# FerrisMind/candle-video

Hardware: AMD Instinct MI355X
Metric: frames/sec end-to-end LTX-Video-2B 512x768x97; DiT step ms; VAE decode ms (higher is better)
Workload: dtype bf16; 1 GPU; LTX-Video-0.9.8-2B-distilled 512x768x97, 7 steps (configs.rs:223-240), untiled VAE decode; preset=0.9.8-2b-distilled, denoise_steps=7, parallelism=replicas x1 (no data-path collective)

## Files before the change

candle-video_amd/csrc/conv_halo.hip:

```cpp
#include <type_traits>
#include "gemm_common.h"
#include "options.h"

#ifndef HALO_WIDE_EPI
#define HALO_WIDE_EPI 1
#endif
#ifndef HALO_LOADERS
#define HALO_LOADERS 4
#endif
#ifndef HALO_PABL
#define HALO_PABL 0
#endif
#ifndef HALO_ABL
#define HALO_ABL 0
#endif

#ifdef HALO_TRACE
__device__ unsigned long long g_halo_trace[16384 * 8];
extern "C" int ltx_dbg_halo_trace(unsigned long long* out, int n) { return hipMemcpyFromSymbol(out, HIP_SYMBOL(g_halo_trace), (size_t)n * 8) == hipSuccess ? 0 : -1; }
#define HSTAMP(i) do { if (threadIdx.x == 0 && blockIdx.x < 16384) g_halo_trace[blockIdx.x * 8 + (i)] = __builtin_amdgcn_s_memrealtime(); } while (0)
#define HCYC(i) do { if (threadIdx.x == 0 && blockIdx.x < 16384) g_halo_trace[blockIdx.x * 8 + (i)] = __builtin_amdgcn_s_memtime(); } while (0)
#else
#define HSTAMP(i) do { } while (0)
#define HCYC(i) do { } while (0)
#endif

namespace {

constexpr int ROWB = 128;
constexpr int PH = 16, PW = 16, HW = PW + 2, HROWS = (PH + 2) * HW;
constexpr int A_PIECES = (HROWS + 7) / 8;
constexpr int A_STAGE = A_PIECES * 1024;
constexpr uint32_t OOB = 0x80000000u;
template <int I, int N, typename F> __device__ __forceinline__ void sfor_h(F&& f) {
    if constexpr (I < N) { f(std::integral_constant<int, I>{}); sfor_h<I + 1, N>(f); }
}

__device__ __forceinline__ int swz_h(int row, int chunk) { return row * ROWB + ((chunk ^ ((row >> 1) & 7)) << 4); }

extern __shared__ __attribute__((aligned(16))) unsigned char halo_smem[];

template <int BN, int WGM, int WGN, int EPI, bool PIPE>
__global__ __launch_bounds__(WGM * WGN * 64) void conv_halo_kernel(const GemmArgs g) {
    constexpr int NW = WGM * WGN, BM = PH * PW, WM = BM / WGM, WN = BN / WGN, FM = WM / 16, FN = BN == 64 ? 3 : WN / 16;
    static_assert((NW == 8 || (NW == 4 && PIPE)) && WM % 16 == 0 && WN % 16 == 0, "wave layout");
    constexpr int NTHR = NW * 64;
    constexpr int NL = (HALO_LOADERS == 4 && (BN == 128 || (BN == 64 && PIPE))) ? 4 : NW;
    constexpr int AJ = (A_PIECES + NL - 1) / NL, BJ = BN / (8 * NL);
    constexpr int B_STAGE = BN * ROWB;
    constexpr int A_ST = PIPE ? AJ * NL * 1024 : A_STAGE;
    static_assert(!PIPE || (NL == 4 && (BN == 128 || BN == 64)), "pipelined form: four loader waves, 128-wide tile (or conv_out's 64-wide one)");
    unsigned char* Abuf = halo_smem;
    unsigned char* Bbuf = halo_smem + 2 * A_ST;
    HSTAMP(0);
#ifndef HALO_NO_KERNARG_BATCH
    asm volatile("" :: "s"(g.A), "s"(g.W), "s"(g.C), "s"(g.bias), "s"(g.resid), "s"(g.N), "s"(g.K), "s"(g.Cin), "s"(g.T), "s"(g.H), "s"(g.Wd), "s"(g.ntaps), "s"(g.pad_t),
                 "s"(g.ldc), "s"(g.ldr), "s"(gridDim.x));
#endif

    const int tid = threadIdx.x, lane = tid & 63, wave = __builtin_amdgcn_readfirstlane(tid >> 6);
    const int wm = wave / WGN, wn = wave % WGN;
    const int lwave = wave & (NL - 1);
    const bool loader = wave < NL;
    const int frow = lane & 15, fq = lane >> 4;

    const int ntn = (g.N + BN - 1) / BN, pwn = (g.Wd + PW - 1) / PW, phn = (g.H + PH - 1) / PH;
    int bid = blockIdx.x;
    {
        const int nblk = (int)gridDim.x, q = nblk >> 3, r = nblk & 7, x = bid & 7, i = bid >> 3;
        bid = (x < r ? x * (q + 1) : r * (q + 1) + (x - r) * q) + i;
    }
#ifdef HALO_SAME_TILE
    bid = bid % ntn;
#endif
    const int nt = bid % ntn; int rr = bid / ntn;
    const int px = rr % pwn; rr /= pwn;
    const int py = rr % phn; const int bt = rr / phn;
    const int t = bt % g.T, b = bt / g.T;
    const int y0 = py * PH, x0 = px * PW, n0 = nt * BN;

    const bf16_t* __restrict__ A = reinterpret_cast<const bf16_t*>(g.A);
    const bf16_t* __restrict__ W = reinterpret_cast<const bf16_t*>(g.W);
    const int64_t frame_elems = (int64_t)g.H * g.Wd * g.Cin;
    const int tt0 = t - g.pad_t < 0 ? 0 : (t - g.pad_t > g.T - 1 ? g.T - 1 : t - g.pad_t);
    const __amdgpu_buffer_rsrc_t ra = __builtin_amdgcn_make_buffer_rsrc(const_cast<bf16_t*>(A + ((int64_t)b * g.T + tt0) * frame_elems), 0, (int)OOB, 0x00020000);
    const __amdgpu_buffer_rsrc_t rw = __builtin_amdgcn_make_buffer_rsrc(const_cast<bf16_t*>(W), 0, (int)OOB, 0x00020000);
    auto dma = [&](__amdgpu_buffer_rsrc_t r, uint32_t voff, uint32_t soff, unsigned char* lds) {
        __builtin_amdgcn_raw_ptr_buffer_load_lds(r, (__attribute__((address_space(3))) void*)lds, 16, (int)voff, (int)soff, 0, 0);
    };

    const int lr = lane >> 3, pc = lane & 7;
    uint32_t a_voff[AJ], b_voff[BJ];
#pragma unroll
    for (int j = 0; j < AJ; ++j) {
        const int hrow = (j * NL + lwave) * 8 + lr;
        const int hy = hrow / HW, hx = hrow - hy * HW;
        const int lc = pc ^ ((hx >> 1) & 7);
        const int y = y0 - 1 + hy, x = x0 - 1 + hx;
        const bool ok = hrow < HROWS && y >= 0 && y < g.H && x >= 0 && x < g.Wd;
        a_voff[j] = ok ? (uint32_t)(((y * g.Wd + x) * g.Cin + lc * 8) * 2) : OOB;
    }
#pragma unroll
    for (int j = 0; j < BJ; ++j) {
        const int row = (j * NL + lwave) * 8 + lr;
        const int lc = pc ^ ((row >> 1) & 7);
        b_voff[j] = n0 + row < g.N ? (uint32_t)((((n0 + row) * g.K) + lc * 8) * 2) : OOB;
    }
    const int KC = g.Cin / 64;
    const int KT = g.ntaps / 9;
    const int G = KT * KC;
    const uint32_t frame_bytes = (uint32_t)g.H * g.Wd * g.Cin * 2u;
    auto issue_a = [&](int grp, int j) {
        const int piece = j * NL + lwave;
        if (!loader || piece >= A_PIECES) return;
        const int it = grp / KC, kc = grp - it * KC;
        int tt = t + it - g.pad_t; tt = tt < 0 ? 0 : (tt > g.T - 1 ? g.T - 1 : tt);
        const uint32_t soff = (uint32_t)(tt - tt0) * frame_bytes + (uint32_t)kc * 128u;
        dma(ra, a_voff[j], soff, Abuf + (grp & 1) * A_ST + piece * 1024);
    };
    auto issue_b = [&](int grp, int hw, int buf) {
        if (!loader) return;
        const int it = grp / KC, kc = grp - it * KC;
        const uint32_t soff = ((uint32_t)(it * 9 + hw) * (uint32_t)g.N * (uint32_t)g.K + (uint32_t)kc * 64u) * 2u;
#pragma unroll
        for (int j = 0; j < BJ; ++j) dma(rw, b_voff[j], soff, Bbuf + buf * B_STAGE + (j * NL + lwave) * 1024);
    };

    f32x4 acc[FM][FN];
#pragma unroll
    for (int i = 0; i < FM; ++i)
#pragma unroll
        for (int j = 0; j < FN; ++j) acc[i][j] = (f32x4){0.f, 0.f, 0.f, 0.f};

    int rowbase[FM], colpart[3][2];
#pragma unroll
    for (int fm = 0; fm < FM; ++fm) rowbase[fm] = ((wm * FM + fm) * HW + frow) * ROWB;
#pragma unroll
    for (int iw = 0; iw < 3; ++iw)
#pragma unroll
        for (int kb = 0; kb < 2; ++kb) colpart[iw][kb] = iw * ROWB + (((kb * 4 + fq) ^ (((frow + iw) >> 1) & 7)) << 4);

    if constexpr (PIPE) {
        auto issue_a_p = [&](int grp, int j) {
            if (!loader) return;
            const int piece = j * NL + lwave;
            const int it = grp / KC, kc = grp - it * KC;
            int tt = t + it - g.pad_t; tt = tt < 0 ? 0 : (tt > g.T - 1 ? g.T - 1 : tt);
            const uint32_t soff = (uint32_t)(tt - tt0) * frame_bytes + (uint32_t)kc * 128u;
            const bool live = grp < G && piece < A_PIECES;
            if ((HALO_PABL & 2) && grp > 0) return;
            dma(ra, live ? a_voff[j] : OOB, live ? soff : 0u, Abuf + (grp & 1) * A_ST + piece * 1024);
        };
        auto issue_b_p = [&](int grp, int hw) {
            if (!loader) return;
            const int it = grp / KC, kc = grp - it * KC;
            const bool live = grp < G;
            const uint32_t soff = live ? ((uint32_t)(it * 9 + hw) * (uint32_t)g.N * (uint32_t)g.K + (uint32_t)kc * 64u) * 2u : 0u;
            if ((HALO_PABL & 2) && (grp > 0 || hw > 1)) return;
#pragma unroll
            for (int j = 0; j < BJ; ++j) dma(rw, live ? b_voff[j] : OOB, soff, Bbuf + (hw % 3) * B_STAGE + (j * NL + lwave) * 1024);
        };
        Chunk16 w0[FN], a0[FM], w1[FN], a1[FM];
        bool frags_once = false;
        auto read_frags = [&](int grp, int hw, int kb, Chunk16 (&wf)[FN], Chunk16 (&af)[FM]) {
            if (HALO_PABL & 4) {
                if (frags_once) {
#pragma unroll
                    for (int f = 0; f < FN; ++f) asm volatile("" : "+v"(wf[f].u));
#pragma unroll
                    for (int f = 0; f < FM; ++f) asm volatile("" : "+v"(af[f].u));
                    return;
                }
            }
            const int ih = hw / 3, iw = hw % 3;
            const unsigned char* As = Abuf + (grp & 1) * A_ST;
            const unsigned char* Bs = Bbuf + (hw % 3) * B_STAGE;
#pragma unroll
            for (int f = 0; f < FN; ++f) wf[f].u = *reinterpret_cast<const u32x4*>(Bs + swz_h(wn * WN + f * 16 + frow, kb * 4 + fq));
#pragma unroll
            for (int fm = 0; fm < FM; ++fm) af[fm].u = *reinterpret_cast<const u32x4*>(As + rowbase[fm] + colpart[iw][kb] + ih * HW * ROWB);
        };
        auto mma_all = [&](Chunk16 (&wf)[FN], Chunk16 (&af)[FM]) {
#pragma unroll
            for (int fm = 0; fm < FM; ++fm)
#pragma unroll
                for (int fn = 0; fn < FN; ++fn) acc[fm][fn] = Mma<bf16_t>::run(wf[fn], af[fm], acc[fm][fn]);
        };
        auto interleave = [&]() {
#pragma unroll
            for (int i = 0; i < FN + FM; ++i) {
                __builtin_amdgcn_sched_group_barrier(0x100, 1, 0);
                __builtin_amdgcn_sched_group_barrier(0x008, FM * FN / (FN + FM), 0);
            }
        };
#pragma unroll
        for (int j = 0; j < AJ; ++j) issue_a_p(0, j);
        issue_b_p(0, 0); issue_b_p(0, 1);
        asm volatile("s_waitcnt vmcnt(0)" ::: "memory");
        __syncthreads();
        HSTAMP(1); HCYC(5);
        read_frags(0, 0, 0, w0, a0);
        if (HALO_PABL & 4) { read_frags(0, 0, 1, w1, a1); frags_once = true; }
        auto step_p = [&](int grp, auto hw_tag) {
            constexpr int hw = decltype(hw_tag)::value;
            constexpr int RPS = (AJ + 5) / 6;
            constexpr int na = (hw + 1) * RPS <= AJ ? RPS : (hw * RPS < AJ ? AJ - hw * RPS : 0);
            if (hw + 2 < 9) issue_b_p(grp, hw + 2); else issue_b_p(grp + 1, hw + 2 - 9);
#pragma unroll
            for (int rr = 0; rr < na; ++rr) issue_a_p(grp + 1, hw * RPS + rr);
            read_frags(grp, hw, 1, w1, a1);
            mma_all(w0, a0);
            interleave();
            if ((HALO_PABL & 9) == 9 || (HALO_PABL & 3) == 3) {}
            else if (HALO_PABL & 1) asm volatile("s_waitcnt vmcnt(%0)" :: "n"(BJ + na) : "memory");
            else if (HALO_PABL & (8 | 2)) asm volatile("s_barrier" ::: "memory");
            else
            asm volatile("s_waitcnt vmcnt(%0)\n\ts_barrier" :: "n"(BJ + na) : "memory");
            if (hw + 1 < 9) read_frags(grp, hw + 1, 0, w0, a0); else read_frags(grp + 1, 0, 0, w0, a0);
            mma_all(w1, a1);
            interleave();
        };
        if constexpr (NW == 4) {
            auto mfma = [&](f32x4& c, const Chunk16& w, const Chunk16& a_) {
                asm volatile("v_mfma_f32_16x16x32_bf16 %0, %1, %2, %0" : "+a"(c) : "v"(w.u), "v"(a_.u));
            };
            const uint32_t nk2 = (uint32_t)g.N * (uint32_t)g.K * 2u;
            auto a_soff_of = [&](int it, int kc) {
                int tt = t + it - g.pad_t; tt = tt < 0 ? 0 : (tt > g.T - 1 ? g.T - 1 : tt);
                return (uint32_t)(tt - tt0) * frame_bytes + (uint32_t)kc * 128u;
            };
            int it_n = KC > 1 ? 0 : 1, kc_n = KC > 1 ? 1 : 0;
            uint32_t w_cur = 0u;
            for (int grp = 0; grp < G; ++grp) {
                const bool live_n = grp + 1 < G;
                const uint32_t a_next = live_n ? a_soff_of(it_n, kc_n) : 0u;
                const uint32_t w_next = live_n ? ((uint32_t)(it_n * 9) * (uint32_t)g.N * (uint32_t)g.K + (uint32_t)kc_n * 64u) * 2u : 0u;
                unsigned char* const a_dst = Abuf + ((grp + 1) & 1) * A_ST;
                sfor_h<0, 9>([&](auto hw_tag) {
                    constexpr int hw = decltype(hw_tag)::value;
                    constexpr int RPS = (AJ + 5) / 6;
                    constexpr int na = (hw + 1) * RPS <= AJ ? RPS : (hw * RPS < AJ ? AJ - hw * RPS : 0);
                    constexpr int NP = BJ + na, NM = FM * FN;
                    constexpr int h2 = hw + 2 < 9 ? hw + 2 : hw + 2 - 9;
                    const bool w_live = hw + 2 < 9 ? true : live_n;
                    const uint32_t w_soff = (hw + 2 < 9 ? w_cur : w_next) + (uint32_t)h2 * nk2;
                    auto read_one = [&](int rg, int rh, int kb, auto idx_tag, Chunk16 (&wf)[FN], Chunk16 (&af)[FM]) {
                        constexpr int idx = decltype(idx_tag)::value;
                        if (HALO_PABL & 4) return;
                        const int ih = rh / 3, iw = rh % 3;
                        if constexpr (idx < FN) wf[idx].u = *reinterpret_cast<const u32x4*>(Bbuf + (rh % 3) * B_STAGE + swz_h(wn * WN + idx * 16 + frow, kb * 4 + fq));
                        else af[idx - FN].u = *reinterpret_cast<const u32x4*>(Abuf + (rg & 1) * A_ST + rowbase[idx - FN] + colpart[iw][kb] + ih * HW * ROWB);
                    };
                    auto piece = [&](auto i_tag) {
                        constexpr int i = decltype(i_tag)::value;
                        if constexpr (i < BJ) {
                            if (!((HALO_PABL & 2) && (grp > 0 || hw > 1)))
                                dma(rw, w_live ? b_voff[i] : OOB, w_live ? w_soff : 0u, Bbuf + (h2 % 3) * B_STAGE + (i * NL + lwave) * 1024);
                        } else {
                            constexpr int j = hw * RPS + (i - BJ);
                            const bool live = live_n && j * NL + lwave < A_PIECES;
                            if (!(HALO_PABL & 2)) dma(ra, live ? a_voff[j] : OOB, live ? a_next : 0u, a_dst + (j * NL + lwave) * 1024);
                        }
                    };
                    sfor_h<0, NM>([&](auto m_tag) {
                        constexpr int mi = decltype(m_tag)::value;
                        if constexpr (mi % 2 == 0 && mi / 2 < FN + FM) read_one(grp, hw, 1, std::integral_constant<int, mi / 2>{}, w1, a1);
                        if constexpr (mi % 2 == 1 && (mi / 2) % (16 / NP > 0 ? 16 / NP : 1) == 0 && (mi / 2) / (16 / NP > 0 ? 16 / NP : 1) < NP)
                            piece(std::integral_constant<int, (mi / 2) / (16 / NP > 0 ? 16 / NP : 1)>{});
                        mfma(acc[mi / FN][mi % FN], w0[mi % FN], a0[mi / FN]);
                        __builtin_amdgcn_sched_barrier(0);
                    });
                    if ((HALO_PABL & 9) == 9 || (HALO_PABL & 3) == 3) {}
                    else if (HALO_PABL & 1) asm volatile("s_waitcnt vmcnt(%0)" :: "n"(BJ + na) : "memory");
                    else if (HALO_PABL & (8 | 2)) asm volatile("s_barrier" ::: "memory");
                    else asm volatile("s_waitcnt vmcnt(%0)\n\ts_barrier" :: "n"(BJ + na) : "memory");
                    __builtin_amdgcn_sched_barrier(0);
                    sfor_h<0, NM>([&](auto m_tag) {
                        constexpr int mi = decltype(m_tag)::value;
                        if constexpr (mi % 2 == 0 && mi / 2 < FN + FM) {
                            if (hw + 1 < 9) read_one(grp, hw + 1, 0, std::integral_constant<int, mi / 2>{}, w0, a0);
                            else read_one(grp + 1, 0, 0, std::integral_constant<int, mi / 2>{}, w0, a0);
                        }
                        mfma(acc[mi / FN][mi % FN], w1[mi % FN], a1[mi / FN]);
                        __builtin_amdgcn_sched_barrier(0);
                    });
                });
                w_cur = w_next;
                if (++kc_n == KC) { kc_n = 0; ++it_n; }
            }
            asm volatile("s_nop 15\n\ts_nop 15" ::: "memory");
        } else
        for (int grp = 0; grp < G; ++grp) {
            step_p(grp, std::integral_constant<int, 0>{}); step_p(grp, std::integral_constant<int, 1>{}); step_p(grp, std::integral_constant<int, 2>{});
            step_p(grp, std::integral_constant<int, 3>{}); step_p(grp, std::integral_constant<int, 4>{}); step_p(grp, std::integral_constant<int, 5>{});
            step_p(grp, std::integral_constant<int, 6>{}); step_p(grp, std::integral_constant<int, 7>{}); step_p(grp, std::integral_constant<int, 8>{});
        }
        HCYC(6); HSTAMP(2);
        asm volatile("s_waitcnt vmcnt(0)" ::: "memory");
        __syncthreads();
    } else {
#pragma unroll
    for (int j = 0; j < AJ; ++j) issue_a(0, j);
    issue_b(0, 0, 0);
    asm volatile("s_waitcnt vmcnt(0)" ::: "memory");
    __syncthreads();

    auto step = [&](int grp, auto hw_tag, int buf) {
        constexpr int hw = decltype(hw_tag)::value;
        constexpr int ih = hw / 3, iw = hw % 3;
        if (!(HALO_ABL & 4)) { if (hw < 8) issue_b(grp, hw + 1, buf ^ 1); else if (grp + 1 < G) issue_b(grp + 1, 0, buf ^ 1); }
        constexpr int RPS = (AJ + 8) / 9;
        if (!(HALO_ABL & 4) && grp + 1 < G) {
#pragma unroll
            for (int rr = 0; rr < RPS; ++rr) if (hw * RPS + rr < AJ) issue_a(grp + 1, hw * RPS + rr);
        }
        const unsigned char* As = Abuf + (grp & 1) * A_ST;
        const unsigned char* Bs = Bbuf + buf * B_STAGE;
#pragma unroll
        for (int kb = 0; kb < 2; ++kb) {
            Chunk16 af[FM], wf[FN];
#pragma unroll
            for (int f = 0; f < FN; ++f) {
                if ((HALO_ABL & 2) && f > 0) { wf[f].u = wf[0].u + (u32x4){(uint32_t)f, 0u, 0u, 0u}; continue; }
                wf[f].u = *reinterpret_cast<const u32x4*>(Bs + swz_h(wn * WN + f * 16 + frow, kb * 4 + fq));
            }
            int fr_ = frow; asm volatile("" : "+v"(fr_));
            const int cp = BN == 256 ? iw * ROWB + (((kb * 4 + fq) ^ (((fr_ + iw) >> 1) & 7)) << 4) : colpart[iw][kb];
            af[0].u = *reinterpret_cast<const u32x4*>(As + rowbase[0] + cp + ih * HW * ROWB);
#pragma unroll
            for (int fm = 0; fm < FM; ++fm) {
                if ((HALO_ABL & 1) && fm + 1 < FM) af[fm + 1].u = af[0].u + (u32x4){(uint32_t)fm, 0u, 0u, 0u};
                else
                if (fm + 1 < FM) af[fm + 1].u = *reinterpret_cast<const u32x4*>(As + rowbase[fm + 1] + cp + ih * HW * ROWB);
#pragma unroll
                for (int fn = 0; fn < FN; ++fn) acc[fm][fn] = Mma<bf16_t>::run(wf[fn], af[fm], acc[fm][fn]);
            }
        }
#pragma unroll
        for (int kb = 0; kb < 2; ++kb) {
            __builtin_amdgcn_sched_group_barrier(0x100, FN + 1, 0);
#pragma unroll
            for (int fm = 0; fm < FM; ++fm) {
                if (fm + 1 < FM) __builtin_amdgcn_sched_group_barrier(0x100, 1, 0);
                __builtin_amdgcn_sched_group_barrier(0x008, FN, 0);
            }
        }
        asm volatile("s_waitcnt vmcnt(0)" ::: "memory");
        __syncthreads();
    };
    for (int grp = 0; grp < G; ++grp) {
        const int p = grp & 1;
        step(grp, std::integral_constant<int, 0>{}, p);
        step(grp, std::integral_constant<int, 1>{}, p ^ 1);
        step(grp, std::integral_constant<int, 2>{}, p);
        step(grp, std::integral_constant<int, 3>{}, p ^ 1);
        step(grp, std::integral_constant<int, 4>{}, p);
        step(grp, std::integral_constant<int, 5>{}, p ^ 1);
        step(grp, std::integral_constant<int, 6>{}, p);
        step(grp, std::integral_constant<int, 7>{}, p ^ 1);
        step(grp, std::integral_constant<int, 8>{}, p);
    }

    }
    constexpr bool WIDE = HALO_WIDE_EPI && (EPI == EPI_BIAS || EPI == EPI_RESID);
    if constexpr (WIDE) {
        if (g.wide_epi) {
            constexpr int CPR = BN / 8, XM = 15, RPP = 64 / CPR;
            const int64_t frame_row0 = ((int64_t)b * g.T + t) * g.H * g.Wd;
            const __amdgpu_buffer_rsrc_t rr = __builtin_amdgcn_make_buffer_rsrc(
                const_cast<bf16_t*>(reinterpret_cast<const bf16_t*>(g.resid ? g.resid : g.C) + frame_row0 * g.ldr), 0, (int)OOB, 0x00020000);
            auto row_m = [&](int row, bool& inside) {
                const int y = y0 + (row >> 4), x = x0 + (row & 15);
                inside = y < g.H && x < g.Wd;
                return ((b * g.T + t) * g.H + y) * g.Wd + x;
            };
            if constexpr (EPI == EPI_RESID) {
                for (int pi = wave; pi < BM / RPP; pi += NW) {
                    const int row = pi * RPP + lane / CPR, pc = lane % CPR;
                    const int lc = pc ^ (row & XM);
                    bool inside; const int m = row_m(row, inside);
                    dma(rr, inside ? (uint32_t)((((int64_t)m - frame_row0) * g.ldr + n0 + lc * 8) * 2) : OOB, 0u, halo_smem + pi * 1024);
                }
                asm volatile("s_waitcnt vmcnt(0)" ::: "memory");
            }
            float bias4[FN][4];
#pragma unroll
            for (int fn = 0; fn < FN; ++fn) {
#pragma unroll
                for (int i = 0; i < 4; ++i) bias4[fn][i] = 0.f;
            }
            if (g.bias) {
#pragma unroll
                for (int fn = 0; fn < FN; ++fn) load4<bf16_t>(reinterpret_cast<const bf16_t*>(g.bias) + n0 + wn * WN + fn * 16 + 4 * fq, bias4[fn]);
            }
            __syncthreads();
#pragma unroll
            for (int fm = 0; fm < FM; ++fm) {
                const int row = (wm * FM + fm) * 16 + frow;
#pragma unroll
                for (int fn = 0; fn < FN; ++fn) {
                    const int col = wn * WN + fn * 16 + 4 * fq;
                    unsigned char* slot = halo_smem + row * (CPR * 16) + (((col >> 3) ^ (row & XM)) << 4) + ((col >> 2) & 1) * 8;
                    float v[4] = {acc[fm][fn][0], acc[fm][fn][1], acc[fm][fn][2], acc[fm][fn][3]};
                    {
#pragma unroll
                        for (int i = 0; i < 4; ++i) v[i] += bias4[fn][i];
                    }
                    if constexpr (EPI == EPI_RESID) {
                        float r[4];
                        load4<bf16_t>(reinterpret_cast<const bf16_t*>(slot), r);
#pragma unroll
                        for (int i = 0; i < 4; ++i) v[i] += r[i];
                    }
                    store4<bf16_t>(reinterpret_cast<bf16_t*>(slot), v);
                }
            }
            __syncthreads();
            bf16_t* Cb = reinterpret_cast<bf16_t*>(g.C);
            float pn_sc[8], pn_sh[8];
            bool pn_mod = false;
            if constexpr (EPI == EPI_BIAS) {
                if (g.pn_on && g.pn_scale) {
                    pn_mod = true;
                    const int c0 = tid % CPR;
                    const f32x4* scp = reinterpret_cast<const f32x4*>(g.pn_scale + (int64_t)b * g.pn_mod_stride + c0 * 8);
                    const f32x4* shp = reinterpret_cast<const f32x4*>(g.pn_shift + (int64_t)b * g.pn_mod_stride + c0 * 8);
                    const f32x4 s0 = scp[0], s1 = scp[1], h0 = shp[0], h1 = shp[1];
#pragma unroll
                    for (int j = 0; j < 4; ++j) { pn_sc[j] = 1.0f + s0[j]; pn_sc[4 + j] = 1.0f + s1[j]; pn_sh[j] = h0[j]; pn_sh[4 + j] = h1[j]; }
                }
            }
            for (int id = tid; id < BM * CPR; id += NTHR) {
                const int row = id / CPR, c = id - row * CPR;
                bool inside; const int m = row_m(row, inside);
                Chunk16 cc; cc.u = *reinterpret_cast<const u32x4*>(halo_smem + row * (CPR * 16) + ((c ^ (row & XM)) << 4));
                if constexpr (EPI == EPI_BIAS) {
                    if (g.pn_on) {
                        float f[8]; chunk_to_f32<bf16_t>(cc, f);
                        float ss = 0.f;
#pragma unroll
                        for (int j = 0; j < 8; ++j) ss += f[j] * f[j];
#pragma unroll
                        for (int o = CPR / 2; o > 0; o >>= 1) ss += __shfl_xor(ss, o);
                        const float rinv = __builtin_amdgcn_rsqf(ss * (1.0f / (float)BN) + g.pn_eps);
#pragma unroll
                        for (int j = 0; j < 8; ++j) {
                            float n = f[j] * rinv;
                            if (pn_mod) n = n * pn_sc[j] + pn_sh[j];
                            if (g.pn_act == 1) n = silu_f(n);
                            f[j] = n;
                        }
                        f32_to_chunk<bf16_t>(f, cc);
                    }
                }
                if (!inside) continue;
                *reinterpret_cast<u32x4*>(Cb + (int64_t)m * g.ldc + n0 + c * 8) = cc.u;
            }
#ifdef HALO_TRACE
            HSTAMP(3); asm volatile("s_waitcnt vmcnt(0)" ::: "memory"); HSTAMP(4);
            if (threadIdx.x == 0 && blockIdx.x < 16384) { unsigned hw; asm volatile("s_getreg_b32 %0, hwreg(HW_REG_HW_ID)" : "=s"(hw)); g_halo_trace[blockIdx.x * 8 + 7] = hw; }
#endif
            return;
        }
    }
    if constexpr (EPI == EPI_S2D) {
        float bias4[FN][4];
#pragma unroll
        for (int fn = 0; fn < FN; ++fn) {
#pragma unroll
            for (int i = 0; i < 4; ++i) bias4[fn][i] = 0.f;
        }
        if (g.bias) {
#pragma unroll
            for (int fn = 0; fn < FN; ++fn) {
                int nb = n0 + wn * WN + fn * 16 + 4 * fq; nb = nb < g.N ? nb : g.N - 4;
                load4<bf16_t>(reinterpret_cast<const bf16_t*>(g.bias) + nb, bias4[fn]);
            }
        }
        const int npass = (t == 0 && g.s2_st > 1) ? 2 : 1;
        for (int pass = 0; pass < npass; ++pass) {
#pragma unroll
            for (int fm = 0; fm < FM; ++fm) {
                int y = y0 + wm * FM + fm, x = x0 + frow;
                const bool inside = y < g.H && x < g.Wd;
                y = y < g.H ? y : g.H - 1; x = x < g.Wd ? x : g.Wd - 1;
                float res[FN][4];
#pragma unroll
                for (int fn = 0; fn < FN; ++fn) {
                    int nb = n0 + wn * WN + fn * 16 + 4 * fq; nb = nb < g.N ? nb : g.N - 4;
                    s2d_residual<bf16_t>(g, b, t, y, x, nb, pass, res[fn]);
                }
                if (!inside) continue;
#pragma unroll
                for (int fn = 0; fn < FN; ++fn) {
                    const int nb = n0 + wn * WN + fn * 16 + 4 * fq;
                    if (nb >= g.N) continue;
                    float v[4];
#pragma unroll
                    for (int i = 0; i < 4; ++i) v[i] = acc[fm][fn][i] + bias4[fn][i];
                    s2d_store<bf16_t>(g, b, t, y, x, nb, pass, v, res[fn]);
                }
            }
        }
    } else if constexpr (EPI == EPI_D2S || EPI == EPI_UNPATCH || EPI == EPI_BIAS || EPI == EPI_D2S_G) {
        float bias4[FN][4];
#pragma unroll
        for (int fn = 0; fn < FN; ++fn) {
            const int nb = n0 + wn * WN + fn * 16 + 4 * fq;
#pragma unroll
            for (int i = 0; i < 4; ++i) bias4[fn][i] = 0.f;
        }
        if (g.bias) {
#pragma unroll
            for (int fn = 0; fn < FN; ++fn) {
                int nb = n0 + wn * WN + fn * 16 + 4 * fq; nb = nb < g.N ? nb : g.N - 4;
                load4<bf16_t>(reinterpret_cast<const bf16_t*>(g.bias) + nb, bias4[fn]);
            }
        }
        const bool d2s_res = EPI == EPI_D2S && g.resid != nullptr;
        GemmArgs gs = g; gs.bias = nullptr; gs.resid = nullptr;
        constexpr int FC = FM * FN > 16 ? 2 : FM;
#pragma unroll
        for (int f0 = 0; f0 < FM; f0 += FC) {
            bf16_t raw[FC][FN][4];
            if constexpr (EPI == EPI_D2S) {
                if (d2s_res) {
                    const int nsub = g.d2s_sp ? 4 : 8;
#pragma unroll
                    for (int fc = 0; fc < FC; ++fc) {
                        int y = y0 + wm * FM + f0 + fc, x = x0 + frow;
                        y = y < g.H ? y : g.H - 1; x = x < g.Wd ? x : g.Wd - 1;
                        const int m = ((b * g.T + t) * g.H + y) * g.Wd + x;
                        const bf16_t* xr = reinterpret_cast<const bf16_t*>(g.resid) + (int64_t)m * g.Cin;
#pragma unroll
                        for (int fn = 0; fn < FN; ++fn) {
                            int nb = n0 + wn * WN + fn * 16 + 4 * fq; nb = nb < g.N ? nb : g.N - 4;
                            const int sidx = nb / g.Cf, co = nb - sidx * g.Cf;
#pragma unroll
                            for (int i = 0; i < 4; ++i) raw[fc][fn][i] = xr[((co + i) % g.Cr) * nsub + sidx];
                        }
                    }
                }
            }
#pragma unroll
            for (int fc = 0; fc < FC; ++fc) {
                const int fm = f0 + fc;
                const int y = y0 + wm * FM + fm, x = x0 + frow;
                if (y >= g.H || x >= g.Wd) continue;
                const int m = ((b * g.T + t) * g.H + y) * g.Wd + x;
#pragma unroll
                for (int fn = 0; fn < FN; ++fn) {
                    const int nb = n0 + wn * WN + fn * 16 + 4 * fq;
                    if (nb >= g.N) continue;
                    float v[4];
#pragma unroll
                    for (int i = 0; i < 4; ++i) v[i] = acc[fm][fn][i] + bias4[fn][i];
                    if constexpr (EPI == EPI_D2S) {
                        if (d2s_res) {
#pragma unroll
                            for (int i = 0; i < 4; ++i) v[i] += to_f32(raw[fc][fn][i]);
                        }
                    }
                    epilogue<bf16_t, EPI>(gs, m, nb, v);
                }
            }
        }
    } else {
#pragma unroll
    for (int fm = 0; fm < FM; ++fm) {
        const int y = y0 + wm * FM + fm, x = x0 + frow;
        if (y >= g.H || x >= g.Wd) continue;
        const int m = ((b * g.T + t) * g.H + y) * g.Wd + x;
#pragma unroll
        for (int fn = 0; fn < FN; ++fn) {
            const int nb = n0 + wn * WN + fn * 16 + 4 * fq;
            if (nb >= g.N) continue;
            float v[4] = {acc[fm][fn][0], acc[fm][fn][1], acc[fm][fn][2], acc[fm][fn][3]};
            epilogue<bf16_t, EPI>(g, m, nb, v);
        }
    }
    }
}

bool halo_wide_epi(const GemmArgs& g) {
    return ltx_opt().gemm_wide_epi && g.ldc % 8 == 0 && ((uintptr_t)g.C & 15) == 0 &&
           (!g.resid || (g.ldr % 8 == 0 && ((uintptr_t)g.resid & 15) == 0 && (double)g.H * g.Wd * g.ldr * 2.0 < 2147483648.0));
}

template <int BN, int WGM, int WGN, int EPI, bool PIPE = false>
int launch_halo(const GemmArgs& g, hipStream_t s) {
    constexpr int smem = PIPE ? 2 * 44 * 1024 + 3 * BN * ROWB : 2 * A_STAGE + 2 * BN * ROWB;
    static std::atomic<unsigned long long> attr_devs{0};
    auto kern = conv_halo_kernel<BN, WGM, WGN, EPI, PIPE>;
    LTX_TRY(ltx_set_max_dyn_smem(attr_devs, reinterpret_cast<const void*>(kern), smem));
    const int tiles = g.B * g.T * cdiv(g.H, PH) * cdiv(g.Wd, PW) * cdiv(g.N, BN);
    GemmArgs ga = g;
    ga.wide_epi = halo_wide_epi(g);
    if (g.pn_on && (!ga.wide_epi || BN != g.N || !ltx_conv_halo_norm_ok(g, EPI))) LTX_FAIL(LTX_ERR_ARG, "conv_halo: the fused output norm needs the wide bias epilogue and BN == N");
    LTX_LAUNCH_TIMED(kern, dim3((unsigned)tiles), dim3(WGM * WGN * 64), smem, s, ga);
    LTX_CHECK_LAUNCH();
    return LTX_OK;
}

template <int BN, int WGM, int WGN, bool PIPE = false>
int launch_halo_epi(const GemmArgs& g, int epi, hipStream_t s) {
    switch (epi) {
        case EPI_BIAS: return launch_halo<BN, WGM, WGN, EPI_BIAS, PIPE>(g, s);
        case EPI_RESID: return launch_halo<BN, WGM, WGN, EPI_RESID, PIPE>(g, s);
        case EPI_D2S: return launch_halo<BN, WGM, WGN, EPI_D2S, PIPE>(g, s);
        case EPI_S2D: return launch_halo<BN, WGM, WGN, EPI_S2D, PIPE>(g, s);
        case EPI_D2S_G: return launch_halo<BN, WGM, WGN, EPI_D2S_G, PIPE>(g, s);
    }
    LTX_FAIL(LTX_ERR_ARG, "conv_halo: unsupported epilogue");
}

}

bool ltx_conv_halo_eligible(const GemmArgs& g, int epi, int bn) {
    if (!g.conv || g.ntaps != 27 || g.kh != 3 || g.kw != 3) return false;
    if (g.Cin % 64 != 0 || g.K != g.Cin) return false;
    if (bn == 64) {
        if (epi != EPI_UNPATCH || g.N > 48 || g.N % 4 != 0) return false;
    } else {
        if (g.N % bn != 0) return false;
        if (epi != EPI_BIAS && epi != EPI_RESID && epi != EPI_D2S && epi != EPI_S2D && epi != EPI_D2S_G) return false;
    }
    if (g.c_seg_shift) return false;
    const double frame_bytes = (double)g.H * g.Wd * g.Cin * 2.0, w_bytes = 27.0 * g.N * g.K * 2.0;
    return 3.0 * frame_bytes < 2147483648.0 && w_bytes < 2147483648.0 && (double)g.B * g.T * g.H * g.Wd < 2147483648.0;
}

bool ltx_conv_halo_norm_ok(const GemmArgs& g, int epi) {
    if (!HALO_WIDE_EPI || epi != EPI_BIAS || (g.N != 128 && g.N != 256) || !halo_wide_epi(g)) return false;
    if ((g.pn_scale == nullptr) != (g.pn_shift == nullptr)) return false;
    if (g.pn_scale && (g.pn_mod_stride % 4 != 0 || (((uintptr_t)g.pn_scale | (uintptr_t)g.pn_shift) & 15))) return false;
    return ltx_conv_halo_eligible(g, epi, g.N);
}

int ltx_launch_conv_halo(const GemmArgs& g, int epi, int bn, hipStream_t s) {
    ltx_prof_kernel(LTX_PROFK_CONV_HALO);
    if (!ltx_conv_halo_eligible(g, epi, bn)) LTX_FAIL(LTX_ERR_ARG, "conv_halo: shape not eligible");
#ifdef HALO_CONV_OUT_PLAIN
    if (bn == 64) return launch_halo<64, 8, 1, EPI_UNPATCH, false>(g, s);
#else
    if (bn == 64) return launch_halo<64, 8, 1, EPI_UNPATCH, true>(g, s);
#endif
    if (bn == 256) return launch_halo_epi<256, 2, 4>(g, epi, s);
#if HALO_LOADERS == 4
#ifdef LTX_EXPERIMENTS
    if (!ltx_exp("conv_halo_pipe", 1)) return launch_halo_epi<128, 4, 2>(g, epi, s);
    if (ltx_exp("conv_halo_w4", 0)) return launch_halo_epi<128, 2, 2, true>(g, epi, s);
#endif
    return launch_halo_epi<128, 4, 2, true>(g, epi, s);
#else
    return launch_halo_epi<128, 4, 2>(g, epi, s);
#endif
}
```

candle-video_amd/csrc/options.cpp:

```cpp
#include "options.h"
#include <atomic>
#include <cstdio>
#include <cstdlib>
#include <cstring>
#include <map>
#include <mutex>
#include <string>
#include "errors.h"

namespace {
std::mutex g_mu;
LtxOptions g_opt;
std::atomic<bool> g_loaded{false};
std::map<std::string, int> g_exp;

struct ListBit { const char* name; unsigned bit; };
const ListBit kFam[] = {{"asm16", LTX_FAM_ASM16}, {"ring", LTX_FAM_RING}, {"p8", LTX_FAM_P8}, {"halo", LTX_FAM_HALO}, {"halo_out", LTX_FAM_HALO_OUT}, {"big", LTX_FAM_BIG}};
const ListBit kAttn[] = {{"q64", LTX_ATTN_Q64}, {"q128", LTX_ATTN_Q128}, {"cross", LTX_ATTN_CROSS}, {"pipe", LTX_ATTN_PIPE}};

template <size_t N> bool parse_list(const char* v, const ListBit (&tab)[N], unsigned* out) {
    unsigned bits = 0;
    std::string s(v ? v : "");
    size_t p = 0;
    while (p < s.size()) {
        size_t q = s.find('+', p); if (q == std::string::npos) q = s.size();
        const std::string item = s.substr(p, q - p);
        bool ok = item.empty();
        for (const auto& t : tab) if (item == t.name) { bits |= t.bit; ok = true; }
        if (!ok) return false;
        p = q + 1;
    }
    *out = bits;
    return true;
}

struct IntField { const char* name; int LtxOptions::*field; };
const IntField kInts[] = {
    {"gemm_tune", &LtxOptions::gemm_tune}, {"gemm_wide_epi", &LtxOptions::gemm_wide_epi}, {"gemm_trace", &LtxOptions::gemm_trace},
    {"attn_q64_big", &LtxOptions::attn_q64_big}, {"vae_tile_batch", &LtxOptions::vae_tile_batch}, {"prof_kernel_events", &LtxOptions::prof_kernel_events}, {"ff2_defer", &LtxOptions::ff2_defer},
    {"gemm_splitk", &LtxOptions::gemm_splitk}, {"q2_fold", &LtxOptions::q2_fold}, {"norm_presum", &LtxOptions::norm_presum}, {"norm_lean", &LtxOptions::norm_lean},
    {"xattn_compact", &LtxOptions::xattn_compact}, {"xattn_fold_vo", &LtxOptions::xattn_fold_vo}, {"dense_qkv", &LtxOptions::dense_qkv}, {"vae_fuse_norm", &LtxOptions::vae_fuse_norm}, {"t5_attn_mfma", &LtxOptions::t5_attn_mfma}, {"guidance_batch", &LtxOptions::guidance_batch}, {"norm_fold", &LtxOptions::norm_fold}, {"norm_fold_copies", &LtxOptions::norm_fold_copies}, {"attn_q64_stream", &LtxOptions::attn_q64_stream},
};

bool set_one(LtxOptions& o, const std::string& key, const char* value) {
    static const LtxOptions dflt;
    for (const auto& f : kInts) if (key == f.name) {
        if (!value) { o.*(f.field) = dflt.*(f.field); return true; }
        char* end = nullptr; const long v = strtol(value, &end, 10);
        if (end == value || *end) return false;
        o.*(f.field) = (int)v; return true;
    }
    if (key == "gemm_plan") {
        if (!value) { o.gemm_plan[0] = 0; return true; }
        if (strlen(value) >= sizeof(o.gemm_plan)) return false;
        strcpy(o.gemm_plan, value); return true;
    }
    if (key == "gemm_off") return value ? parse_list(value, kFam, &o.gemm_off) : (o.gemm_off = 0, true);
    if (key == "attn_off") return value ? parse_list(value, kAttn, &o.attn_off) : (o.attn_off = 0, true);
    if (key.rfind("x_", 0) == 0) {
        if (!value) { g_exp.erase(key); return true; }
        char* end = nullptr; const long v = strtol(value, &end, 10);
        if (end == value || *end) return false;
        g_exp[key] = (int)v; return true;
    }
    return false;
}

bool parse_string(LtxOptions& o, const char* text, std::string* bad) {
    std::string s(text ? text : "");
    size_t p = 0;
    while (p < s.size()) {
        size_t q = s.find(',', p); if (q == std::string::npos) q = s.size();
        const std::string item = s.substr(p, q - p);
        p = q + 1;
        if (item.empty()) continue;
        const size_t eq = item.find('=');
        if (eq == std::string::npos || !set_one(o, item.substr(0, eq), item.c_str() + eq + 1)) { if (bad) *bad = item; return false; }
    }
    return true;
}

void load_locked() {
    g_opt = LtxOptions(); g_exp.clear();
    std::string bad;
    if (!parse_string(g_opt, getenv("LTX_OPTIONS"), &bad))
        fprintf(stderr, "[ltx] LTX_OPTIONS: entry '%s' not understood (see include/ltxhip.h); it and what follows it are ignored\n", bad.c_str());
    g_loaded.store(true, std::memory_order_release);
}
}

const LtxOptions& ltx_opt() {
    if (!g_loaded.load(std::memory_order_acquire)) { std::lock_guard<std::mutex> lock(g_mu); if (!g_loaded.load(std::memory_order_relaxed)) load_locked(); }
    return g_opt;
}

int ltx_exp_lookup(const char* name, int dflt) {
    (void)ltx_opt();
    std::lock_guard<std::mutex> lock(g_mu);
    auto it = g_exp.find(std::string("x_") + name);
    return it == g_exp.end() ? dflt : it->second;
}

extern "C" int ltx_set_option(const char* key, const char* value) {
    if (!key) LTX_FAIL(LTX_ERR_ARG, "ltx_set_option: null key");
    (void)ltx_opt();
    std::lock_guard<std::mutex> lock(g_mu);
    if (!set_one(g_opt, key, value)) LTX_FAIL(LTX_ERR_ARG, std::string("ltx_set_option: unknown option or bad value: ") + key + "=" + (value ? value : "(default)"));
    return LTX_OK;
}

extern "C" int ltx_get_option(const char* key, char* out, int n) {
    if (!key || !out || n < 2) LTX_FAIL(LTX_ERR_ARG, "ltx_get_option: null key / buffer");
    (void)ltx_opt();
    std::lock_guard<std::mutex> lock(g_mu);
    const std::string k(key);
    std::string v; bool found = false;
    for (const auto& f : kInts) if (k == f.name) { v = std::to_string(g_opt.*(f.field)); found = true; }
    auto list = [&](unsigned bits, const ListBit* tab, size_t cnt) { for (size_t i = 0; i < cnt; ++i) if (bits & tab[i].bit) { if (!v.empty()) v += "+"; v += tab[i].name; } found = true; };
    if (k == "gemm_plan") { v = g_opt.gemm_plan; found = true; }
    if (k == "gemm_off") list(g_opt.gemm_off, kFam, sizeof(kFam) / sizeof(kFam[0]));
    if (k == "attn_off") list(g_opt.attn_off, kAttn, sizeof(kAttn) / sizeof(kAttn[0]));
    if (k.rfind("x_", 0) == 0) { auto it = g_exp.find(k); if (it == g_exp.end()) LTX_FAIL(LTX_ERR_ARG, "ltx_get_option: experiment knob not set: " + k); v = std::to_string(it->second); found = true; }
    if (!found) LTX_FAIL(LTX_ERR_ARG, "ltx_get_option: unknown option: " + k);
    if ((int)v.size() + 1 > n) LTX_FAIL(LTX_ERR_ARG, "ltx_get_option: buffer too small");
    memcpy(out, v.c_str(), v.size() + 1);
    return LTX_OK;
}

extern "C" int ltx_reset_options(void) {
    std::lock_guard<std::mutex> lock(g_mu);
    load_locked();
    return LTX_OK;
}

extern "C" int ltx_has_experiments(void) {
#ifdef LTX_EXPERIMENTS
    return 1;
#else
    return 0;
#endif
}
```

candle-video_amd/csrc/options.h:

```cpp
#pragma once

enum { LTX_FAM_ASM16 = 1, LTX_FAM_RING = 2, LTX_FAM_P8 = 4, LTX_FAM_HALO = 8, LTX_FAM_HALO_OUT = 16, LTX_FAM_BIG = 32 };
enum { LTX_ATTN_Q64 = 1, LTX_ATTN_Q128 = 2, LTX_ATTN_CROSS = 4, LTX_ATTN_PIPE = 8 };

struct LtxOptions {
    int gemm_tune = 1;
    char gemm_plan[40] = {0};
    unsigned gemm_off = 0;
    int gemm_wide_epi = 1;
    int gemm_trace = 0;
    int attn_q64_big = -1;
    int vae_tile_batch = 0;
    int prof_kernel_events = 1;
    int ff2_defer = 1;
    int gemm_splitk = 1;
    int q2_fold = 1;
    int norm_presum = 1;
    int norm_lean = 1;
    int xattn_compact = 1;
    int xattn_fold_vo = 1;
    int attn_q64_stream = 0;
    int norm_fold = 2;
    int norm_fold_copies = 10;
    int guidance_batch = 1;
    int dense_qkv = 1;
    int vae_fuse_norm = 1;
    int t5_attn_mfma = 1;
    unsigned attn_off = 0;
};

const LtxOptions& ltx_opt();
int ltx_exp_lookup(const char* name, int dflt);
#ifdef LTX_EXPERIMENTS
#define ltx_exp(name, dflt) ltx_exp_lookup(name, dflt)
#else
#define ltx_exp(name, dflt) (dflt)
#endif
```

Measured before the change: 574.0 frames/sec.

## Add half-patch pair variant of halo conv for two workgroups per CU

Adds a conv_halo kernel variant that covers an 8-row half patch with 2x2 waves and fits two workgroups per CU by halving the LDS footprint. It uses its own double-buffered schedule for weights and activations, with a barrier at each tap. It is enabled by default for bias and residual epilogues when Cin is at least 512 and the tile count is large. The aim is better latency hiding through more occupancy, at the cost of more halo reloads per output row and more barriers.

Result: no change. 573.6 frames/sec (median of 2 runs) (-0.1%).

```diff
diff --git a/candle-video_amd/csrc/conv_halo.hip b/candle-video_amd/csrc/conv_halo.hip
--- a/candle-video_amd/csrc/conv_halo.hip
+++ b/candle-video_amd/csrc/conv_halo.hip
@@ -40,15 +40,18 @@
 
 extern __shared__ __attribute__((aligned(16))) unsigned char halo_smem[];
 
-template <int BN, int WGM, int WGN, int EPI, bool PIPE>
-__global__ __launch_bounds__(WGM * WGN * 64) void conv_halo_kernel(const GemmArgs g) {
-    constexpr int NW = WGM * WGN, BM = PH * PW, WM = BM / WGM, WN = BN / WGN, FM = WM / 16, FN = BN == 64 ? 3 : WN / 16;
+template <int BN, int WGM, int WGN, int EPI, bool PIPE, int PHT = PH>
+__global__ __launch_bounds__(WGM * WGN * 64, PHT == PH ? 1 : 2) void conv_halo_kernel(const GemmArgs g) {
+    constexpr bool PAIR = PHT != PH;
+    constexpr int HROWS = (PHT + 2) * HW, A_PIECES = (HROWS + 7) / 8, A_STAGE = A_PIECES * 1024;
+    constexpr int NW = WGM * WGN, BM = PHT * PW, WM = BM / WGM, WN = BN / WGN, FM = WM / 16, FN = BN == 64 ? 3 : WN / 16;
     static_assert((NW == 8 || (NW == 4 && PIPE)) && WM % 16 == 0 && WN % 16 == 0, "wave layout");
+    static_assert(!PAIR || (PHT == 8 && BN == 128 && WGM == 2 && WGN == 2 && PIPE), "pair form: half a patch, 2 x 2 waves of 64 x 64");
     constexpr int NTHR = NW * 64;
     constexpr int NL = (HALO_LOADERS == 4 && (BN == 128 || (BN == 64 && PIPE))) ? 4 : NW;
     constexpr int AJ = (A_PIECES + NL - 1) / NL, BJ = BN / (8 * NL);
     constexpr int B_STAGE = BN * ROWB;
-    constexpr int A_ST = PIPE ? AJ * NL * 1024 : A_STAGE;
+    constexpr int A_ST = PIPE && !PAIR ? AJ * NL * 1024 : A_STAGE;
     static_assert(!PIPE || (NL == 4 && (BN == 128 || BN == 64)), "pipelined form: four loader waves, 128-wide tile (or conv_out's 64-wide one)");
     unsigned char* Abuf = halo_smem;
     unsigned char* Bbuf = halo_smem + 2 * A_ST;
@@ -64,7 +67,7 @@
     const bool loader = wave < NL;
     const int frow = lane & 15, fq = lane >> 4;
 
-    const int ntn = (g.N + BN - 1) / BN, pwn = (g.Wd + PW - 1) / PW, phn = (g.H + PH - 1) / PH;
+    const int ntn = (g.N + BN - 1) / BN, pwn = (g.Wd + PW - 1) / PW, phn = (g.H + PHT - 1) / PHT;
     int bid = blockIdx.x;
     {
         const int nblk = (int)gridDim.x, q = nblk >> 3, r = nblk & 7, x = bid & 7, i = bid >> 3;
@@ -77,7 +80,7 @@
     const int px = rr % pwn; rr /= pwn;
     const int py = rr % phn; const int bt = rr / phn;
     const int t = bt % g.T, b = bt / g.T;
-    const int y0 = py * PH, x0 = px * PW, n0 = nt * BN;
+    const int y0 = py * PHT, x0 = px * PW, n0 = nt * BN;
 
     const bf16_t* __restrict__ A = reinterpret_cast<const bf16_t*>(g.A);
     const bf16_t* __restrict__ W = reinterpret_cast<const bf16_t*>(g.W);
@@ -193,9 +196,23 @@
                 __builtin_amdgcn_sched_group_barrier(0x008, FM * FN / (FN + FM), 0);
             }
         };
+        const uint32_t nk2_q = (uint32_t)g.N * (uint32_t)g.K * 2u;
+        auto a_soff_q = [&](int it, int kc) {
+            int tt = t + it - g.pad_t; tt = tt < 0 ? 0 : (tt > g.T - 1 ? g.T - 1 : tt);
+            return (uint32_t)(tt - tt0) * frame_bytes + (uint32_t)kc * 128u;
+        };
+        if constexpr (PAIR) {
+#pragma unroll
+            for (int j = 0; j < AJ; ++j) if (j * NL + lwave < A_PIECES) dma(ra, a_voff[j], a_soff_q(0, 0), Abuf + (j * NL + lwave) * 1024);
+#pragma unroll
+            for (int h = 0; h < 2; ++h)
+#pragma unroll
+                for (int j = 0; j < BJ; ++j) dma(rw, b_voff[j], (uint32_t)h * nk2_q, Bbuf + h * B_STAGE + (j * NL + lwave) * 1024);
+        } else {
 #pragma unroll
         for (int j = 0; j < AJ; ++j) issue_a_p(0, j);
         issue_b_p(0, 0); issue_b_p(0, 1);
+        }
         asm volatile("s_waitcnt vmcnt(0)" ::: "memory");
         __syncthreads();
         HSTAMP(1); HCYC(5);
@@ -220,7 +237,49 @@
             mma_all(w1, a1);
             interleave();
         };
-        if constexpr (NW == 4) {
+        if constexpr (PAIR) {
+            auto read_q = [&](int abuf, int hw, int slot, int kb, Chunk16 (&wf)[FN], Chunk16 (&af)[FM]) {
+                const int ih = hw / 3, iw = hw % 3;
+                const unsigned char* As = Abuf + abuf * A_ST;
+                const unsigned char* Bs = Bbuf + slot * B_STAGE;
+#pragma unroll
+                for (int f = 0; f < FN; ++f) wf[f].u = *reinterpret_cast<const u32x4*>(Bs + swz_h(wn * WN + f * 16 + frow, kb * 4 + fq));
+#pragma unroll
+                for (int fm = 0; fm < FM; ++fm) af[fm].u = *reinterpret_cast<const u32x4*>(As + rowbase[fm] + colpart[iw][kb] + ih * HW * ROWB);
+            };
+            int it_n = KC > 1 ? 0 : 1, kc_n = KC > 1 ? 1 : 0;
+            uint32_t w_cur = 0u;
+            for (int grp = 0; grp < G; ++grp) {
+                const bool live_n = grp + 1 < G;
+                const uint32_t a_next = live_n ? a_soff_q(it_n, kc_n) : 0u;
+                const uint32_t w_next = live_n ? ((uint32_t)(it_n * 9) * (uint32_t)g.N * (uint32_t)g.K + (uint32_t)kc_n * 64u) * 2u : 0u;
+                unsigned char* const a_dst = Abuf + ((grp + 1) & 1) * A_ST;
+                const int par = grp & 1;
+                sfor_h<0, 9>([&](auto hw_tag) {
+                    constexpr int hw = decltype(hw_tag)::value;
+                    constexpr int h2 = hw + 2 < 9 ? hw + 2 : hw + 2 - 9;
+                    const int slot = par ^ (hw & 1);
+                    const bool w_live = hw + 2 < 9 ? true : live_n;
+                    const uint32_t w_soff = (hw + 2 < 9 ? w_cur : w_next) + (uint32_t)h2 * nk2_q;
+                    read_q(par, hw, slot, 1, w1, a1);
+                    mma_all(w0, a0);
+                    interleave();
+                    asm volatile("s_waitcnt vmcnt(0) lgkmcnt(0)\n\ts_barrier" ::: "memory");
+                    if (w_live) {
+#pragma unroll
+                        for (int j = 0; j < BJ; ++j) dma(rw, b_voff[j], w_soff, Bbuf + slot * B_STAGE + (j * NL + lwave) * 1024);
+                    }
+                    if constexpr (hw < AJ) {
+                        if (live_n && hw * NL + lwave < A_PIECES) dma(ra, a_voff[hw], a_next, a_dst + (hw * NL + lwave) * 1024);
+                    }
+                    if (hw + 1 < 9) read_q(par, hw + 1, slot ^ 1, 0, w0, a0); else read_q(par ^ 1, 0, slot ^ 1, 0, w0, a0);
+                    mma_all(w1, a1);
+                    interleave();
+                });
+                w_cur = w_next;
+                if (++kc_n == KC) { kc_n = 0; ++it_n; }
+            }
+        } else if constexpr (NW == 4) {
             auto mfma = [&](f32x4& c, const Chunk16& w, const Chunk16& a_) {
                 asm volatile("v_mfma_f32_16x16x32_bf16 %0, %1, %2, %0" : "+a"(c) : "v"(w.u), "v"(a_.u));
             };
@@ -587,13 +646,18 @@
            (!g.resid || (g.ldr % 8 == 0 && ((uintptr_t)g.resid & 15) == 0 && (double)g.H * g.Wd * g.ldr * 2.0 < 2147483648.0));
 }
 
-template <int BN, int WGM, int WGN, int EPI, bool PIPE = false>
+std::atomic<long long> g_pair_launches{0};
+
+template <int BN, int WGM, int WGN, int EPI, bool PIPE = false, int PHT = PH>
 int launch_halo(const GemmArgs& g, hipStream_t s) {
-    constexpr int smem = PIPE ? 2 * 44 * 1024 + 3 * BN * ROWB : 2 * A_STAGE + 2 * BN * ROWB;
+    constexpr bool PAIR = PHT != PH;
+    constexpr int smem = PAIR ? 2 * (((PHT + 2) * HW + 7) / 8) * 1024 + 2 * BN * ROWB : PIPE ? 2 * 44 * 1024 + 3 * BN * ROWB : 2 * A_STAGE + 2 * BN * ROWB;
+    static_assert(!PAIR || smem <= 80 * 1024, "pair form: two workgroups share a CU's 160 KiB of LDS");
     static std::atomic<unsigned long long> attr_devs{0};
-    auto kern = conv_halo_kernel<BN, WGM, WGN, EPI, PIPE>;
+    auto kern = conv_halo_kernel<BN, WGM, WGN, EPI, PIPE, PHT>;
     LTX_TRY(ltx_set_max_dyn_smem(attr_devs, reinterpret_cast<const void*>(kern), smem));
-    const int tiles = g.B * g.T * cdiv(g.H, PH) * cdiv(g.Wd, PW) * cdiv(g.N, BN);
+    const int tiles = g.B * g.T * cdiv(g.H, PHT) * cdiv(g.Wd, PW) * cdiv(g.N, BN);
+    if (PAIR) g_pair_launches.fetch_add(1, std::memory_order_relaxed);
     GemmArgs ga = g;
     ga.wide_epi = halo_wide_epi(g);
     if (g.pn_on && (!ga.wide_epi || BN != g.N || !ltx_conv_halo_norm_ok(g, EPI))) LTX_FAIL(LTX_ERR_ARG, "conv_halo: the fused output norm needs the wide bias epilogue and BN == N");
@@ -614,6 +678,37 @@
     LTX_FAIL(LTX_ERR_ARG, "conv_halo: unsupported epilogue");
 }
 
+constexpr int kPairMinTiles = 512, kPairMinCin = 512;
+bool halo_pair_serves(int epi) { return epi == EPI_BIAS || epi == EPI_RESID || epi == EPI_D2S; }
+bool halo_pair_rule(const GemmArgs& g, int epi) {
+    const int mode = ltx_opt().conv_halo_pair;
+    if (mode <= 0 || !halo_pair_serves(epi)) return false;
+    if (mode >= 2) return true;
+    const int64_t tiles = (int64_t)g.B * g.T * cdiv(g.H, PH) * cdiv(g.Wd, PW) * cdiv(g.N, 128);
+    return epi != EPI_D2S && g.Cin >= kPairMinCin && tiles >= kPairMinTiles;
+}
+int launch_halo_pair(const GemmArgs& g, int epi, hipStream_t s) {
+    switch (epi) {
+        case EPI_BIAS: return launch_halo<128, 2, 2, EPI_BIAS, true, 8>(g, s);
+        case EPI_RESID: return launch_halo<128, 2, 2, EPI_RESID, true, 8>(g, s);
+        case EPI_D2S: return launch_halo<128, 2, 2, EPI_D2S, true, 8>(g, s);
+    }
+    LTX_FAIL(LTX_ERR_ARG, "conv_halo: the pair form does not serve this epilogue");
+}
+
+}
+
+extern "C" long long ltx_dbg_halo_pair(int what, int epi) {
+    if (what == 0) return g_pair_launches.load(std::memory_order_relaxed);
+    if (what != 1 || !halo_pair_serves(epi)) return -1;
+    constexpr int smem = 2 * (((8 + 2) * HW + 7) / 8) * 1024 + 2 * 128 * ROWB;
+    const void* k = epi == EPI_BIAS ? reinterpret_cast<const void*>(conv_halo_kernel<128, 2, 2, EPI_BIAS, true, 8>)
+                  : epi == EPI_RESID ? reinterpret_cast<const void*>(conv_halo_kernel<128, 2, 2, EPI_RESID, true, 8>)
+                                     : reinterpret_cast<const void*>(conv_halo_kernel<128, 2, 2, EPI_D2S, true, 8>);
+    static std::atomic<unsigned long long> attr_devs{0};
+    if (ltx_set_max_dyn_smem(attr_devs, k, smem) != LTX_OK) return -1;
+    int n = 0;
+    return hipOccupancyMaxActiveBlocksPerMultiprocessor(&n, k, 256, smem) == hipSuccess ? n : -1;
 }
 
 bool ltx_conv_halo_eligible(const GemmArgs& g, int epi, int bn) {
@@ -651,6 +746,7 @@
     if (!ltx_exp("conv_halo_pipe", 1)) return launch_halo_epi<128, 4, 2>(g, epi, s);
     if (ltx_exp("conv_halo_w4", 0)) return launch_halo_epi<128, 2, 2, true>(g, epi, s);
 #endif
+    if (halo_pair_rule(g, epi)) return launch_halo_pair(g, epi, s);
     return launch_halo_epi<128, 4, 2, true>(g, epi, s);
 #else
     return launch_halo_epi<128, 4, 2>(g, epi, s);
diff --git a/candle-video_amd/csrc/options.cpp b/candle-video_amd/csrc/options.cpp
--- a/candle-video_amd/csrc/options.cpp
+++ b/candle-video_amd/csrc/options.cpp
@@ -39,7 +39,7 @@
     {"gemm_tune", &LtxOptions::gemm_tune}, {"gemm_wide_epi", &LtxOptions::gemm_wide_epi}, {"gemm_trace", &LtxOptions::gemm_trace},
     {"attn_q64_big", &LtxOptions::attn_q64_big}, {"vae_tile_batch", &LtxOptions::vae_tile_batch}, {"prof_kernel_events", &LtxOptions::prof_kernel_events}, {"ff2_defer", &LtxOptions::ff2_defer},
     {"gemm_splitk", &LtxOptions::gemm_splitk}, {"q2_fold", &LtxOptions::q2_fold}, {"norm_presum", &LtxOptions::norm_presum}, {"norm_lean", &LtxOptions::norm_lean},
-    {"xattn_compact", &LtxOptions::xattn_compact}, {"xattn_fold_vo", &LtxOptions::xattn_fold_vo}, {"dense_qkv", &LtxOptions::dense_qkv}, {"vae_fuse_norm", &LtxOptions::vae_fuse_norm}, {"t5_attn_mfma", &LtxOptions::t5_attn_mfma}, {"guidance_batch", &LtxOptions::guidance_batch}, {"norm_fold", &LtxOptions::norm_fold}, {"norm_fold_copies", &LtxOptions::norm_fold_copies}, {"attn_q64_stream", &LtxOptions::attn_q64_stream},
+    {"xattn_compact", &LtxOptions::xattn_compact}, {"xattn_fold_vo", &LtxOptions::xattn_fold_vo}, {"dense_qkv", &LtxOptions::dense_qkv}, {"vae_fuse_norm", &LtxOptions::vae_fuse_norm}, {"t5_attn_mfma", &LtxOptions::t5_attn_mfma}, {"guidance_batch", &LtxOptions::guidance_batch}, {"norm_fold", &LtxOptions::norm_fold}, {"norm_fold_copies", &LtxOptions::norm_fold_copies}, {"attn_q64_stream", &LtxOptions::attn_q64_stream}, {"conv_halo_pair", &LtxOptions::conv_halo_pair},
 };
 
 bool set_one(LtxOptions& o, const std::string& key, const char* value) {
diff --git a/candle-video_amd/csrc/options.h b/candle-video_amd/csrc/options.h
--- a/candle-video_amd/csrc/options.h
+++ b/candle-video_amd/csrc/options.h
@@ -11,6 +11,7 @@
     int gemm_trace = 0;
     int attn_q64_big = -1;
     int vae_tile_batch = 0;
+    int conv_halo_pair = 1;
     int prof_kernel_events = 1;
     int ff2_defer = 1;
     int gemm_splitk = 1;
```
